# yeyupiaoling/VoiceprintRecognition-PaddlePaddle

Measured on NVIDIA H100. Metric: utterances/sec ECAPA-TDNN Fbank80 3s embed extract, higher is better.
Workload: dtype bf16x3 (split-bf16 operands, fp32 accumulate; fp32-grade)

## Files before the change

voiceprintrecognition-paddlepaddle_b200/csrc/asp_fused.cu:

```cuda
#include <stdio.h>
#include <string.h>

#include "common.h"
#include "ptx.cuh"

namespace ppv {

constexpr int AF_NT = 64;
constexpr int AF_A_TILE = 128 * 64 * 2;
constexpr int AF_B_TILE = AF_NT * 64 * 2;
constexpr int AF_X_TILE = AF_NT * 128 * 2;
constexpr int AF_STAGES = 2;
constexpr float LOG2E = 1.4426950408889634f;

template <int NSPLIT>
__global__ void __launch_bounds__(384, 1) asp_fused_kernel(const __grid_constant__ AspFusedParams p) {
    constexpr int NP = (NSPLIT == 3) ? 2 : 1;
    extern __shared__ uint8_t smem_raw[];
    const uint32_t smem_base = (smem_u32(smem_raw) + 1023u) & ~1023u;
    uint8_t* smem_gen = smem_raw + (smem_base - smem_u32(smem_raw));
    const int ksteps = p.K / 64;
    const int a_bytes = ksteps * NP * AF_A_TILE;
    const int b_bytes = ksteps * NP * AF_B_TILE;
    const int stage_bytes = b_bytes + 2 * AF_X_TILE;
    const uint32_t a_base = smem_base;
    const uint32_t s_base = smem_base + a_bytes;
    const uint32_t bar_base = s_base + AF_STAGES * stage_bytes;
    const uint32_t a_full = bar_base, a_empty = bar_base + 8;
    auto b_full = [&](int s) { return bar_base + 16u + 8u * s; };
    auto b_empty = [&](int s) { return bar_base + 32u + 8u * s; };

    const int warp = threadIdx.x >> 5, lane = threadIdx.x & 31;
    if (warp == 0 && lane == 0) {
        prefetch_tmap(&p.mapW);
        prefetch_tmap(&p.mapAtt);
        prefetch_tmap(&p.mapX);
    }
    if (warp == 1 && lane == 0) {
        mbar_init(a_full, 1);
        mbar_init(a_empty, 256);
        for (int s = 0; s < AF_STAGES; ++s) {
            mbar_init(b_full(s), 1);
            mbar_init(b_empty(s), 256);
        }
        fence_mbar_init();
    }
    __syncthreads();
    griddep_launch_dependents();
    griddep_wait();

    const int slabs = p.C / 128;
    const int items = slabs * p.B;
    const int ntiles = (p.T + AF_NT - 1) / AF_NT;

    if (warp == 0) {
        int stage = 0;
        uint32_t phase = 0, a_phase = 0;
        int cur_slab = -1;
        for (int item = blockIdx.x; item < items; item += gridDim.x) {
            const int b = item / slabs, slab = item - b * slabs;
            if (slab != cur_slab) {
                mbar_wait(a_empty, a_phase ^ 1u);
                if (lane == 0) {
                    mbar_arrive_expect_tx(a_full, a_bytes);
                    for (int ks = 0; ks < ksteps; ++ks)
                        for (int pl = 0; pl < NP; ++pl)
                            tma_load_3d(a_base + (ks * NP + pl) * AF_A_TILE, &p.mapW, a_full, ks * 64, slab * 128, pl);
                }
                __syncwarp();
                a_phase ^= 1u;
                cur_slab = slab;
            }
            {
                const int nitem = item + gridDim.x;
                if (nitem < items && lane < 2 * ntiles) {
                    const int nb = nitem / slabs, nslab = nitem - nb * slabs;
                    tma_prefetch_l2_3d(&p.mapX, nslab * 128, nb * p.Tp + p.P + (lane >> 1) * AF_NT, lane & 1);
                }
                __syncwarp();
            }
            const int row0 = b * p.Tp + p.P;
            for (int ft = 0; ft < ntiles; ++ft) {
                mbar_wait(b_empty(stage), phase ^ 1u);
                if (lane == 0) {
                    const uint32_t sb = s_base + stage * stage_bytes;
                    mbar_arrive_expect_tx(b_full(stage), stage_bytes);
                    for (int ks = 0; ks < ksteps; ++ks)
                        for (int pl = 0; pl < NP; ++pl)
                            tma_load_3d(sb + (ks * NP + pl) * AF_B_TILE, &p.mapAtt, b_full(stage), ks * 64, row0 + ft * AF_NT, pl);
                    for (int pl = 0; pl < 2; ++pl)
                        tma_load_3d(sb + b_bytes + pl * AF_X_TILE, &p.mapX, b_full(stage), slab * 128, row0 + ft * AF_NT, pl);
                }
                __syncwarp();
                if (++stage == AF_STAGES) {
                    stage = 0;
                    phase ^= 1u;
                }
            }
        }
    } else if (warp >= 4) {
        const int g = (warp - 4) >> 2, t = threadIdx.x & 127, w = t >> 5, l = t & 31;
        const int cl0 = 64 * g + 16 * w + (l >> 2);
        float acc[AF_NT / 2];
#pragma unroll
        for (int i = 0; i < AF_NT / 2; ++i) acc[i] = 0.f;
        int stage = 0;
        uint32_t phase = 0, a_phase = 0;
        int cur_slab = -1;
        for (int item = blockIdx.x; item < items; item += gridDim.x) {
            const int b = item / slabs, slab = item - b * slabs;
            if (slab != cur_slab) {
                mbar_wait(a_full, a_phase);
                a_phase ^= 1u;
                cur_slab = slab;
            }
            const int nitem = item + gridDim.x;
            const bool last_of_slab = (nitem >= items) || (nitem % slabs != slab);
            float m[2], S0[2], mu[2], M2[2];
#pragma unroll
            for (int rr = 0; rr < 2; ++rr) {
                m[rr] = -INFINITY;
                S0[rr] = mu[rr] = M2[rr] = 0.f;
            }
            const int Tb = p.nvalid ? max(1, min(p.T, p.nvalid[b])) : p.T;
            for (int ft = 0; ft < ntiles; ++ft) {
                mbar_wait(b_full(stage), phase);
                const uint32_t sb = s_base + stage * stage_bytes;
                wgmma_fence_acc(acc);
                wgmma_fence();
                for (int ks = 0; ks < ksteps; ++ks) {
                    const uint64_t a_hi = make_sw128_kmajor_desc(a_base + (ks * NP) * AF_A_TILE + g * 64 * 128);
                    const uint64_t b_hi = make_sw128_kmajor_desc(sb + (ks * NP) * AF_B_TILE);
#pragma unroll
                    for (int k = 0; k < 4; ++k) wgmma_bf16<AF_NT>(acc, a_hi + 2 * k, b_hi + 2 * k, (ks > 0 || k > 0) ? 1u : 0u);
                    if (NSPLIT == 3) {
                        const uint64_t a_lo = make_sw128_kmajor_desc(a_base + (ks * NP + 1) * AF_A_TILE + g * 64 * 128);
                        const uint64_t b_lo = make_sw128_kmajor_desc(sb + (ks * NP + 1) * AF_B_TILE);
#pragma unroll
                        for (int k = 0; k < 4; ++k) wgmma_bf16<AF_NT>(acc, a_lo + 2 * k, b_hi + 2 * k, 1u);
#pragma unroll
                        for (int k = 0; k < 4; ++k) wgmma_bf16<AF_NT>(acc, a_hi + 2 * k, b_lo + 2 * k, 1u);
                    }
                }
                wgmma_commit();
                wgmma_wait<0>();
                wgmma_fence_acc(acc);
                if (ft == ntiles - 1 && last_of_slab) mbar_arrive(a_empty);
                const __nv_bfloat16* xs_hi = reinterpret_cast<const __nv_bfloat16*>(smem_gen + (sb - smem_base) + b_bytes);
                const __nv_bfloat16* xs_lo = xs_hi + AF_X_TILE / 2;
                const int f0 = ft * AF_NT;
#pragma unroll
                for (int rr = 0; rr < 2; ++rr) {
                    float cm = -INFINITY;
#pragma unroll
                    for (int i = 0; i < AF_NT / 8; ++i)
#pragma unroll
                        for (int e = 0; e < 2; ++e)
                            if (f0 + 8 * i + 2 * (l & 3) + e < Tb) cm = fmaxf(cm, acc[4 * i + 2 * rr + e]);
                    if (cm > m[rr]) {
                        const float r = exp2f((m[rr] - cm) * LOG2E);
                        S0[rr] *= r;
                        M2[rr] *= r;
                        m[rr] = cm;
                    }
                    const float ms = m[rr] * LOG2E;
                    const int cl = cl0 + 8 * rr;
                    const float x0 = __bfloat162float(xs_hi[2 * (l & 3) * 128 + cl]) + __bfloat162float(xs_lo[2 * (l & 3) * 128 + cl]);
                    float xr[AF_NT / 8][2];
                    float wt = 0.f, sx = 0.f;
#pragma unroll
                    for (int i = 0; i < AF_NT / 8; ++i)
#pragma unroll
                        for (int e = 0; e < 2; ++e) {
                            const int fl = 8 * i + 2 * (l & 3) + e;
                            if (f0 + fl < Tb) {
                                const int o = fl * 128 + cl;
                                xr[i][e] = __bfloat162float(xs_hi[o]) + __bfloat162float(xs_lo[o]);
                                const float ev = exp2f(fmaf(acc[4 * i + 2 * rr + e], LOG2E, -ms));
                                acc[4 * i + 2 * rr + e] = ev;
                                wt += ev;
                                sx = fmaf(ev, xr[i][e] - x0, sx);
                            }
                        }
                    if (wt > 0.f) {
                        const float mt = x0 + sx / wt;
                        float m2 = 0.f;
#pragma unroll
                        for (int i = 0; i < AF_NT / 8; ++i)
#pragma unroll
                            for (int e = 0; e < 2; ++e)
                                if (f0 + 8 * i + 2 * (l & 3) + e < Tb) {
                                    const float d = xr[i][e] - mt;
                                    m2 = fmaf(acc[4 * i + 2 * rr + e] * d, d, m2);
                                }
                        const float n = S0[rr] + wt, f = wt / n, dl = mt - mu[rr];
                        mu[rr] = fmaf(dl, f, mu[rr]);
                        M2[rr] += m2 + dl * dl * (S0[rr] * f);
                        S0[rr] = n;
                    }
                }
                mbar_arrive(b_empty(stage));
                if (++stage == AF_STAGES) {
                    stage = 0;
                    phase ^= 1u;
                }
            }
#pragma unroll
            for (int rr = 0; rr < 2; ++rr) {
#pragma unroll
                for (int off = 1; off <= 2; off <<= 1) {
                    const float om = __shfl_xor_sync(0xffffffffu, m[rr], off), o0 = __shfl_xor_sync(0xffffffffu, S0[rr], off),
                                omu = __shfl_xor_sync(0xffffffffu, mu[rr], off), o2 = __shfl_xor_sync(0xffffffffu, M2[rr], off);
                    const float mm = fmaxf(m[rr], om);
                    const float ra = S0[rr] > 0.f ? exp2f((m[rr] - mm) * LOG2E) : 0.f, rb = o0 > 0.f ? exp2f((om - mm) * LOG2E) : 0.f;
                    const float wa = S0[rr] * ra, wb = o0 * rb, n = wa + wb;
                    const float f = n > 0.f ? wb / n : 0.f, dl = omu - mu[rr];
                    mu[rr] = fmaf(dl, f, mu[rr]);
                    M2[rr] = M2[rr] * ra + o2 * rb + dl * dl * (wa * f);
                    S0[rr] = n;
                    m[rr] = mm;
                }
            }
            if ((l & 3) != 0) continue;
            const int C = p.C;
#pragma unroll
            for (int rr = 0; rr < 2; ++rr) {
                const int c = slab * 128 + cl0 + 8 * rr;
                const float mean = mu[rr];
                const float sd = sqrtf(fmaxf(M2[rr] / S0[rr], p.eps));
                if (p.out_raw) {
                    p.out_raw[int64_t(b) * 2 * C + c] = mean;
                    p.out_raw[int64_t(b) * 2 * C + C + c] = sd;
                }
                __nv_bfloat16 h, lo;
                split_bf16(fmaf(mean, p.bn_scale[c], p.bn_shift[c]), h, lo);
                p.out.hi()[int64_t(b) * p.out.ld + c] = h;
                p.out.lo()[int64_t(b) * p.out.ld + c] = lo;
                split_bf16(fmaf(sd, p.bn_scale[C + c], p.bn_shift[C + c]), h, lo);
                p.out.hi()[int64_t(b) * p.out.ld + C + c] = h;
                p.out.lo()[int64_t(b) * p.out.ld + C + c] = lo;
            }
        }
    }
}

int asp_fused_build(AspFusedParams* p, const Planes& W, const Planes& att, const Planes& x, const float* bn_scale,
                    const float* bn_shift, const Planes& out, float* out_raw, int B, int T, int P, int Tp, int C, int K, float eps) {
    PPV_REQUIRE(C % 128 == 0 && K % 64 == 0 && K <= 128, "asp_fused: C % 128 == 0 and K in {64,128} required");
    memset(p, 0, sizeof(*p));
    PPV_REQUIRE(x.ld == C, "asp_fused: x row length must equal C");
    int rc = encode_planes_map(&p->mapW, W, 128);
    if (rc) return rc;
    rc = encode_planes_map(&p->mapAtt, att, AF_NT);
    if (rc) return rc;
    rc = encode_planes_map_ex(&p->mapX, x, 128, AF_NT, 0);
    if (rc) return rc;
    p->x = x;
    p->bn_scale = bn_scale;
    p->bn_shift = bn_shift;
    p->out = out;
    p->out_raw = out_raw;
    p->B = B;
    p->T = T;
    p->P = P;
    p->Tp = Tp;
    p->C = C;
    p->K = K;
    p->eps = eps;
    p->nvalid = nullptr;
    return PPV_OK;
}

int asp_fused_launch(const AspFusedParams& p, int precision, int num_sms, cudaStream_t st) {
    const bool x3 = precision == PPV_PREC_BF16X3;
    const int ksteps = p.K / 64, np = x3 ? 2 : 1;
    const int smem = 1024 + ksteps * np * AF_A_TILE + AF_STAGES * (ksteps * np * AF_B_TILE + 2 * AF_X_TILE) + 96 + 128 * 16 + 64;
    static bool attr3 = false, attr1 = false;
    bool& attr = x3 ? attr3 : attr1;
    if (!attr) {
        if (x3)
            PPV_CUDA_OK(cudaFuncSetAttribute(asp_fused_kernel<3>, cudaFuncAttributeMaxDynamicSharedMemorySize, 227 * 1024));
        else
            PPV_CUDA_OK(cudaFuncSetAttribute(asp_fused_kernel<1>, cudaFuncAttributeMaxDynamicSharedMemorySize, 227 * 1024));
        attr = true;
    }
    const int items = (p.C / 128) * p.B;
    const int grid = std::min(items, num_sms);
    if (x3)
        PPV_PDL_OK(launch_pdl(asp_fused_kernel<3>, dim3(grid), dim3(384), size_t(smem), st, p), "asp_fused_kernel");
    else
        PPV_PDL_OK(launch_pdl(asp_fused_kernel<1>, dim3(grid), dim3(384), size_t(smem), st, p), "asp_fused_kernel");
    return PPV_OK;
}

}
```

voiceprintrecognition-paddlepaddle_b200/csrc/capi.cu:

```cuda
#include <string.h>

#include <new>

#include "common.h"
#include "image_plan.h"
#include "model_common.h"

namespace ppv {

static thread_local std::string g_last_error;

void set_error(const std::string& msg) { g_last_error = msg; }
int fail(int code, const std::string& msg) {
    g_last_error = msg;
    return code;
}

int device_sm_count() {
    int dev = 0, n = 0;
    if (cudaGetDevice(&dev) != cudaSuccess || cudaDeviceGetAttribute(&n, cudaDevAttrMultiProcessorCount, dev) != cudaSuccess || n <= 0) {
        cudaGetLastError();
        return 132;
    }
    return n;
// ... 469 lines not shown
    rc = gemm_test_stage(A, W, M, N, K, ws, st, &pa, &pw);
    if (rc) return rc;
    GemmSource src{pa, 0, pa.ld, 0};
    const Planes po{static_cast<__nv_bfloat16*>(out), 0, N, int64_t(M) * N};
    Epilogue ep = Tp > 0 ? planes_epilogue(po, 0, Tp, P, Tp - 2 * P) : planes_epilogue(po);
    ep.bias = bias;
    ep.rowgrp_bias = rowgrp_bias;
    ep.relu = relu;
    ep.tanh_ = tanh_;
    ep.bn_scale = bn_scale;
    ep.bn_shift = bn_shift;
    GemmParams gp;
    rc = gemm_build(&gp, &src, 1, pw, M, N, ep, block_n, 64);
    if (rc) return rc;
    return gemm_launch(gp, precision, device_sm_count(), st);
    PPV_GUARD_END
}

static size_t conv2d_test_x_bytes(int B, int H, int W, int x_ld) {
    return au(au(size_t(B) * (H + 2) * (W + 2), 128) * size_t(x_ld) * 4, 256);
}
size_t ppv_conv2d_test_workspace_bytes(int B, int H, int W, int Cin, int Cout, int k, int x_ld) {
    if (x_ld <= 0) x_ld = Cin;
    return conv2d_test_x_bytes(B, H, W, x_ld) + au(au(size_t(Cout), 256) * k * k * Cin * 4, 256) + 256;
}
int ppv_conv2d_test(const float* x, const float* w, const float* bias, int relu, int B, int H, int W, int Cin, int Cout, int k,
                    int stride_h, int stride_w, int x_col0, int x_ld, int path, int precision, void* out, void* ws, size_t ws_bytes,
                    void* stream) {
    PPV_GUARD_BEGIN
    PPV_REQUIRE(x && w && out && ws, "ppv_conv2d_test: null argument");
    if (x_ld <= 0) x_ld = Cin;
    PPV_REQUIRE(B > 0 && H > 0 && W > 0 && Cin > 0 && Cout > 0 && (k == 1 || k == 3) && stride_h >= 1 && stride_w >= 1,
                "ppv_conv2d_test: bad shape");
    PPV_REQUIRE(x_col0 >= 0 && x_col0 + Cin <= x_ld, "ppv_conv2d_test: the input columns exceed x_ld");
    PPV_REQUIRE(path >= 0 && path <= 2, "ppv_conv2d_test: path must be 0 (3x3 patch kernel), 1 (pointwise kernel) or 2 (gather-GEMM)");
    PPV_REQUIRE(precision == PPV_PREC_BF16X3 || precision == PPV_PREC_BF16, "ppv_conv2d_test: bad precision");
    PPV_REQUIRE(ws_bytes >= ppv_conv2d_test_workspace_bytes(B, H, W, Cin, Cout, k, x_ld), "ppv_conv2d_test: workspace too small");
    const int Hp = H + 2, Wp = W + 2, Ho = (H - 1) / stride_h + 1, Wo = (W - 1) / stride_w + 1;
    const int64_t M = int64_t(B) * Hp * Wp;
    PPV_REQUIRE(M < (int64_t(1) << 31) && Wp + 1 < 32768, "ppv_conv2d_test: grid too large for 32-bit rows / 16-bit tap offsets");
    int rc = check_device();
    if (rc) return rc;
    cudaStream_t st = static_cast<cudaStream_t>(stream);
    Planes xp;
    xp.rows = int64_t(au(size_t(M), 128));
    xp.ld = x_ld;
    xp.plane_stride = xp.rows * x_ld;
    xp.base = static_cast<__nv_bfloat16*>(ws);
    const size_t x_bytes = conv2d_test_x_bytes(B, H, W, x_ld);
    PPV_CUDA_OK(cudaMemsetAsync(ws, 0, x_bytes, st));
    const size_t pitch = size_t(x_ld) * sizeof(__nv_bfloat16), rows2 = size_t(2 * xp.rows);
    if (x_col0 > 0) PPV_CUDA_OK(cudaMemset2DAsync(xp.base, pitch, 0x3f, size_t(x_col0) * sizeof(__nv_bfloat16), rows2, st));
    if (x_col0 + Cin < x_ld)
        PPV_CUDA_OK(cudaMemset2DAsync(xp.base + x_col0 + Cin, pitch, 0x3f, size_t(x_ld - x_col0 - Cin) * sizeof(__nv_bfloat16), rows2, st));
    for (int b = 0; b < B; ++b)
        for (int h = 0; h < H; ++h) {
            Planes row = xp;
            row.base = xp.base + ((int64_t(b) * Hp + h + 1) * Wp + 1) * x_ld + x_col0;
            rc = launch_f32_to_planes(x + (int64_t(b) * H + h) * W * Cin, W, Cin, row, st);
            if (rc) return rc;
        }
    const int K = k * k * Cin;
    std::vector<float> wh(size_t(Cout) * K);
    PPV_CUDA_OK(cudaMemcpyAsync(wh.data(), w, wh.size() * sizeof(float), cudaMemcpyDeviceToHost, st));
    PPV_CUDA_OK(cudaStreamSynchronize(st));
    ArenaBuilder ab;
    GemmWeights gw;
    ab.put_matrix(&gw, conv_weight_matrix(wh.data(), Cout, Cin, k * k, Cout, {{k * k, Cin, 0, Cin, 0}}), Cout, K);
    uint8_t* wdev = static_cast<uint8_t*>(ws) + x_bytes;
    PPV_CUDA_OK(cudaMemcpyAsync(wdev, ab.host.data(), ab.host.size(), cudaMemcpyHostToDevice, st));
    PPV_CUDA_OK(cudaStreamSynchronize(st));
    gw.W.base = reinterpret_cast<__nv_bfloat16*>(wdev + ab.patches[0].off);
    const int64_t out_plane = int64_t(B) * (Ho + 2) * (Wo + 2) * Cout;
    PPV_CUDA_OK(cudaMemsetAsync(out, 0, size_t(2 * out_plane) * sizeof(__nv_bfloat16), st));
    Planes outp;
    outp.base = static_cast<__nv_bfloat16*>(out);
    outp.ld = Cout;
    outp.plane_stride = out_plane;
    const ImageGeo gin{H, W, Hp, Wp}, gout{Ho, Wo, Ho + 2, Wo + 2};
    Epilogue ep = image_epilogue(outp, gin, gout, stride_h, stride_w);
    ep.bias = bias;
    ep.relu = relu ? 1 : 0;
    const int sms = device_sm_count();
    if (path == 0) {
        PPV_REQUIRE(k == 3 && conv3x3_c32_supported(Cin, Cout, H, W), "ppv_conv2d_test: the patch kernel takes 3x3 convs with 32 -> 32 channels only");
        Conv3x3Params cp;
        rc = conv3x3_build(&cp, xp, x_col0, gw.W, B, H, W, Hp, Wp, ep);
        if (rc) return rc;
        return conv3x3_launch(cp, precision, sms, st);
    }
    if (path == 1) {
        PPV_REQUIRE(k == 1, "ppv_conv2d_test: the pointwise kernel takes 1x1 convs only");
        const GemmSource src{xp, x_col0, Cin, 0};
        PwStep s;
        if (!pointwise_step_build(&s, &src, 1, gw.W, Cout, M, ep))
            return fail(PPV_EINVAL, "ppv_conv2d_test: the pointwise kernel does not take this conv (or PPV_POINTWISE=0)");
        return pointwise_launch(s, sms, st);
    }
    std::vector<GemmSource> srcs;
    if (k == 3)
        image_taps(&srcs, xp, x_col0, Cin, gin);
    else
        srcs.push_back(GemmSource{xp, x_col0, Cin, 0});
    GemmParams gp;
    rc = gemm_build(&gp, srcs.data(), int(srcs.size()), gw.W, int(M), Cout, ep, gemm_pick_bn(Cout));
    if (rc) return rc;
    return gemm_launch(gp, precision, sms, st);
    PPV_GUARD_END
}

static size_t asp_test_sizes(int B, int Tp, int C, int K, size_t* off) {
    const size_t rows = size_t(B) * Tp + 64;
    const size_t sz[4] = {size_t(C) * K, rows * K, rows * C, size_t(B) * 2 * C};
    size_t o = 0;
    for (int i = 0; i < 4; ++i) {
        off[i] = o;
        o += au(2 * sz[i] * sizeof(__nv_bfloat16), 256);
    }
    return o;
}
size_t ppv_asp_fused_test_workspace_bytes(int B, int Tp, int C, int K) {
    size_t off[4];
    return asp_test_sizes(B, Tp, C, K, off);
}
int ppv_asp_fused_test(const float* W, const float* att, const float* x, const float* bn_scale, const float* bn_shift,
                       const int* nvalid, int B, int T, int P, int Tp, int C, int K, int precision, int max_ctas, float* out_raw,
                       float* out, void* ws, size_t ws_bytes, void* stream) {
    PPV_GUARD_BEGIN
    PPV_REQUIRE(W && att && x && bn_scale && bn_shift && out_raw && out && ws, "ppv_asp_fused_test: null argument");
    PPV_REQUIRE(B > 0 && T > 0 && P >= 0 && Tp >= T + 2 * P && max_ctas >= 0, "ppv_asp_fused_test: bad shape");
    PPV_REQUIRE(precision == PPV_PREC_BF16X3 || precision == PPV_PREC_BF16, "ppv_asp_fused_test: bad precision");
    size_t off[4];
    PPV_REQUIRE(ws_bytes >= asp_test_sizes(B, Tp, C, K, off), "ppv_asp_fused_test: workspace too small");
    int rc = check_device();
    if (rc) return rc;
    cudaStream_t st = static_cast<cudaStream_t>(stream);
    uint8_t* w8 = static_cast<uint8_t*>(ws);
    const int64_t rows = int64_t(B) * Tp;
    auto planes = [&](int i, int64_t nrows, int ld, int64_t alloc_rows) {
        return Planes{reinterpret_cast<__nv_bfloat16*>(w8 + off[i]), nrows, ld, alloc_rows * ld};
    };
    const Planes pw = planes(0, C, K, C), pa = planes(1, rows, K, rows + 64), px = planes(2, rows, C, rows + 64),
                 po = planes(3, B, 2 * C, B);
    PPV_CUDA_OK(cudaMemsetAsync(w8 + off[1], 0x46, off[3] - off[1], st));
    if ((rc = launch_f32_to_planes(W, C, K, pw, st)) || (rc = launch_f32_to_planes(att, rows, K, pa, st)) ||
        (rc = launch_f32_to_planes(x, rows, C, px, st)))
        return rc;
    AspFusedParams ap;
    rc = asp_fused_build(&ap, pw, pa, px, bn_scale, bn_shift, po, out_raw, B, T, P, Tp, C, K, 1e-12f);
    if (rc) return rc;
    ap.nvalid = nvalid;
    rc = asp_fused_launch(ap, precision, max_ctas > 0 ? max_ctas : device_sm_count(), st);
    if (rc) return rc;
    return launch_planes_to_f32(po, 0, 2 * C, B, 1, 0, 1, out, st);
    PPV_GUARD_END
}

int ppv_gemm_bench(int M, int N, int K, int block_n, int block_k, int precision, int planes_out, int iters, void* ws, size_t ws_bytes,
                   float* ms_per_launch, void* stream) {
    PPV_GUARD_BEGIN
    PPV_REQUIRE(ws && ms_per_launch && iters > 0, "ppv_gemm_bench: bad argument");
    PPV_REQUIRE(planes_out >= 0 && planes_out <= 3, "ppv_gemm_bench: planes_out must be 0-3");
    constexpr int kTp = 306, kP = 4;
    PPV_REQUIRE(planes_out < 2 || M % kTp == 0, "ppv_gemm_bench: model epilogues need M % 306 == 0");
    cudaStream_t st = static_cast<cudaStream_t>(stream);
    const size_t Kp = au(size_t(K), 64);
    const size_t a_bytes = au(au(size_t(M), 128) * Kp * 4, 256), w_bytes = au(au(size_t(N), 256) * Kp * 4, 256);
    const size_t o_bytes = au(au(size_t(M), 128) * size_t(N) * 4, 256);
    const size_t v_bytes = au((3 + size_t(M / kTp)) * size_t(N) * 4, 256);
    PPV_REQUIRE(ws_bytes >= a_bytes + w_bytes + o_bytes + v_bytes, "ppv_gemm_bench: workspace too small");
    Planes pa, pw, po;
    pa.rows = int64_t(au(size_t(M), 128)); pa.ld = int(Kp); pa.plane_stride = pa.rows * pa.ld; pa.base = static_cast<__nv_bfloat16*>(ws);
    pw.rows = int64_t(au(size_t(N), 256)); pw.ld = int(Kp); pw.plane_stride = pw.rows * pw.ld;
    pw.base = reinterpret_cast<__nv_bfloat16*>(static_cast<uint8_t*>(ws) + a_bytes);
    po.rows = pa.rows; po.ld = N; po.plane_stride = po.rows * po.ld;
    po.base = reinterpret_cast<__nv_bfloat16*>(static_cast<uint8_t*>(ws) + a_bytes + w_bytes);
    PPV_CUDA_OK(cudaMemsetAsync(ws, 0x11, a_bytes + w_bytes, st));
    float* vec = reinterpret_cast<float*>(static_cast<uint8_t*>(ws) + a_bytes + w_bytes + o_bytes);
    PPV_CUDA_OK(cudaMemsetAsync(vec, 0x3c, v_bytes, st));
    GemmSource src{pa, 0, int(Kp), 0};
    Epilogue ep;
    if (planes_out >= 2) {
        ep = planes_epilogue(po, 0, kTp, kP, kTp - 2 * kP);
        ep.bias = vec; ep.bn_scale = vec + N; ep.bn_shift = vec + 2 * N;
        if (planes_out == 3) { ep.rowgrp_bias = vec + 3 * N; ep.tanh_ = 1; }
    } else if (planes_out) {
        ep = planes_epilogue(po);
    } else {
        ep.out_mode = OUT_F32; ep.out = po.base; ep.out_ld = N;
    }
    ep.relu = 1;
    GemmParams gp;
    int rc = gemm_build(&gp, &src, 1, pw, M, N, ep, block_n, block_k);
    if (rc) return rc;
    const int sms = device_sm_count();
    for (int i = 0; i < 3; ++i) { rc = gemm_launch(gp, precision, sms, st); if (rc) return rc; }
    cudaEvent_t e0, e1;
    PPV_CUDA_OK(cudaEventCreate(&e0));
    PPV_CUDA_OK(cudaEventCreate(&e1));
    PPV_CUDA_OK(cudaEventRecord(e0, st));
    for (int i = 0; i < iters; ++i) { rc = gemm_launch(gp, precision, sms, st); if (rc) return rc; }
    PPV_CUDA_OK(cudaEventRecord(e1, st));
    PPV_CUDA_OK(cudaEventSynchronize(e1));
    float ms = 0.f;
    PPV_CUDA_OK(cudaEventElapsedTime(&ms, e0, e1));
    cudaEventDestroy(e0);
    cudaEventDestroy(e1);
    gemm_trace_dump(gp);
    *ms_per_launch = ms / float(iters);
    return PPV_OK;
    PPV_GUARD_END
}

}
```

voiceprintrecognition-paddlepaddle_b200/csrc/common.h:

```cpp
#pragma once
#include <cuda.h>
#include <cuda_bf16.h>
#include <cuda_runtime.h>
#include <stdint.h>
#include <stdlib.h>

#include <algorithm>
#include <string>
#include <utility>

#include "../../include/ppv_b200.h"

namespace ppv {

void set_error(const std::string& msg);
int fail(int code, const std::string& msg);

#define PPV_CUDA_OK(expr)                                                                             \
    do {                                                                                              \
        cudaError_t _e = (expr);                                                                      \
        if (_e != cudaSuccess)                                                                        \
            return ::ppv::fail(PPV_ECUDA, std::string(#expr) + ": " + cudaGetErrorString(_e));        \
    } while (0)
#define PPV_LAUNCH_OK(what)                                                                           \
// ... 74 lines not shown
    const float* bias = nullptr;
    const float* rowgrp_bias = nullptr;
    const float* bn_scale = nullptr;
    const float* bn_shift = nullptr;
    int relu = 0;
    int tanh_ = 0;
    int sigmoid_ = 0;
    int silu_ = 0;
    float relu_max = 0.f;
    int out_mode = OUT_PLANES;
    void* out = nullptr;
    int64_t out_ld = 0;
    int64_t out_plane_stride = 0;
    int out_col0 = 0;
    int Tp = 0, P = 0, T = 0;
    int halo = 0;
    int img_Hp = 0, img_Wp = 0, img_H = 0, img_W = 0, img_stride = 1, out_Hp = 0, out_Wp = 0;
    int img_stride_w = 0;
    const float* seg_scale = nullptr;
    int seg_len = 0, nseg = 0;
    int zero_invalid = 0;
    int f32_vec_ok = 0;
    int debug_nostore = 0;
    int lean = 0;
};

inline Epilogue planes_epilogue(const Planes& out, int col0 = 0, int Tp = 0, int P = 0, int T = 0) {
    Epilogue ep;
    ep.out_mode = OUT_PLANES;
    ep.out = out.base;
    ep.out_ld = out.ld;
    ep.out_plane_stride = out.plane_stride;
    ep.out_col0 = col0;
    ep.Tp = Tp;
    ep.P = P;
    ep.T = T;
    return ep;
}

constexpr int GEMM_TRACE_TILES = 16;
constexpr int GEMM_TRACE_EVENTS = 16;

struct GemmParams {
    CUtensorMap mapA[GEMM_MAX_MAPS];
    CUtensorMap mapB;
    KStep ksteps[GEMM_MAX_KSTEPS];
    int num_ksteps;
    int bk;
    int ws;
    int lin_splits;
    int lin_b_row0, lin_b_col0;
    int64_t lin_split_rows;
    int M, N;
    int m_tiles, n_tiles;
    Epilogue epi;
    unsigned long long* trace;
    int trace_cta;
    int bn;
};
void gemm_trace_dump(const GemmParams& gp);

struct GemmSource {
    Planes t;
    int col0;
    int ncols;
    int row_off;
};

int gemm_build(GemmParams* gp, const GemmSource* srcs, int nsrc, const Planes& W, int M, int N, const Epilogue& epi,
               int BN, int BK = 0);
int gemm_build_wgrad(GemmParams* gp, const Planes& At, const Planes& Bt, int M, int N, int b_row0, int b_col0, int splits, float* out,
                     int64_t out_ld, int out_col0, int64_t split_rows, int BN);
int gemm_launch(const GemmParams& gp, int precision, int num_sms, cudaStream_t stream);
inline int gemm_pick_bn(int N, int max_bn = 256) {
    for (int bn = max_bn; bn > 64; bn /= 2)
        if (N % bn == 0) return bn;
    return 64;
}

int encode_planes_map(CUtensorMap* m, const Planes& t, int box_rows);
int encode_planes_map_ex(CUtensorMap* m, const Planes& t, int box_cols, int box_rows, int swizzle_bytes);

struct Res2Params {
    CUtensorMap mapA[2];
    CUtensorMap mapW;
    int a_col[2];
    int nsrc, dil;
    int l2_prefetch;
    int M, m_tiles;
    Epilogue epi;
};
int res2conv_build(Res2Params* rp, const GemmSource* srcs, int nsrc, const Planes& W, int M, int dil, const Epilogue& epi);
int res2conv_launch(const Res2Params& rp, int precision, int num_sms, cudaStream_t st);

struct Conv3x3Params {
    CUtensorMap mapX;
    CUtensorMap mapW;
    int x_col0;
    int B, H, W, Hp, Wp;
    int nph, npw, patches;
    Epilogue epi;
};
bool conv3x3_c32_supported(int Cin, int Cout, int H, int W);
int conv3x3_build(Conv3x3Params* cp, const Planes& x, int x_col0, const Planes& Wt, int B, int H, int W, int Hp, int Wp, const Epilogue& epi);
int conv3x3_launch(const Conv3x3Params& cp, int precision, int num_sms, cudaStream_t st);

constexpr int RES2CHAIN_MAX = 7;
struct Res2ChainParams {
    CUtensorMap mapX;
    CUtensorMap mapXt, mapY, mapYtail;
    CUtensorMap mapW[RES2CHAIN_MAX];
    const float* bias[RES2CHAIN_MAX];
    const float* bn_scale[RES2CHAIN_MAX];
    const float* bn_shift[RES2CHAIN_MAX];
    Planes x;
    Planes y;
    int nconv, width, B, T, P, Tp, dil, ntiles;
    int paired;
    unsigned long long* trace;
};
int res2chain_build(Res2ChainParams* cp, const Planes& x, const Planes& y, const Planes* W, const float* const* bias, const float* const* bn_scale,
                    const float* const* bn_shift, int nconv, int B, int T, int P, int Tp, int dil, bool paired);
int res2chain_launch(const Res2ChainParams& cp, int precision, int num_sms, cudaStream_t st);
bool res2chain_fits(int T, int P);
bool res2chain_pair_fits(int T, int P);
void res2chain_trace_dump(const Res2ChainParams& cp);

int pointwise_launch(const GemmSource* srcs, int nsrc, const Planes& W, int64_t M, int N, const Epilogue& ep, int num_sms, cudaStream_t st);
struct PwStep {
    GemmSource srcs[2];
    int nsrc = 0, N = 0;
    int64_t M = 0;
    Planes W;
    Epilogue ep;
};
inline int pointwise_launch(const PwStep& s, int num_sms, cudaStream_t st) { return pointwise_launch(s.srcs, s.nsrc, s.W, s.M, s.N, s.ep, num_sms, st); }
bool pointwise_step_build(PwStep* s, const GemmSource* srcs, int nsrc, const Planes& W, int N, int64_t M, const Epilogue& ep);

bool skinny_linear_supported(int M, int N, int K, const Epilogue& ep);
int skinny_linear_launch(const Planes& x, int x_col0, const Planes& W, int M, int N, int K, const Epilogue& ep, cudaStream_t st);

struct AspFusedParams {
    CUtensorMap mapW;
    CUtensorMap mapAtt;
    CUtensorMap mapX;
    Planes x;
    const float* bn_scale;
    const float* bn_shift;
    Planes out;
    float* out_raw;
    int B, T, P, Tp, C, K;
    float eps;
    const int* nvalid;
};

int asp_fused_build(AspFusedParams* p, const Planes& W, const Planes& att, const Planes& x, const float* bn_scale,
                    const float* bn_shift, const Planes& out, float* out_raw, int B, int T, int P, int Tp, int C, int K, float eps);
int asp_fused_launch(const AspFusedParams& p, int precision, int num_sms, cudaStream_t st);

int launch_pack_features(const float* feat, int B, int T, int F, const Planes& out, int P, int Tp, cudaStream_t st);
int launch_colstats(const Planes& x, int col0, int C, int B, int T, int P, int Tp, int mode, float eps, float* out_f32,
                    const Planes& out_pl, cudaStream_t st, float inv_count = 0.f, const int* nvalid = nullptr);
int launch_lengths_to_counts(const float* lengths, int B, int T, int* nvalid, cudaStream_t st);
int launch_se_scale_res(const Planes& z, const float* scale, const Planes& res, int rc0, const Planes& out, int oc0, int C,
                        int Tp, int64_t rows, int num_sms, cudaStream_t st, int relu = 0, float relu_max = 0.f);
int launch_asp_pool(const float* logits, int64_t lg_ld, const Planes& x, int C, int B, int T, int P, int Tp, float eps,
                    const float* bn_scale, const float* bn_shift, const Planes& out_pl, float* out_raw, cudaStream_t st);
int launch_planes_to_f32(const Planes& x, int col0, int C, int B, int T, int P, int Tp, float* out, cudaStream_t st);
int launch_f32_to_planes(const float* src, int64_t rows, int cols, const Planes& out, cudaStream_t st);

struct Fbank;
int fbank_create(const ppv_fbank_cfg* cfg, Fbank** out);
void fbank_destroy(Fbank* h);
int fbank_num_frames(const Fbank* h, int L);
int fbank_n_mels(const Fbank* h);
int fbank_run(Fbank* h, const float* wav, const float* lens_ratio, int B, int L, float* raw, float* out_f32,
              const Planes& out_pl, int P, int Tp, cudaStream_t st, const int* valid_frames = nullptr);

size_t audio_prep_workspace_bytes(int B, int max_new_len);
int audio_prep(const float* wav, int64_t wav_ld, const int32_t* iparams, const float* fparams, const float* noise, int B, int max_new_len,
               float target_db, int normalize, int Lout, float* out, void* ws, size_t ws_bytes, cudaStream_t st);
size_t audio_prep_reverb_workspace_bytes(int B, int max_new_len, int max_rir_len);
int audio_prep_reverb(const float* wav, int64_t wav_ld, const int32_t* iparams, const float* fparams, const float* noise, const float* rir_bank,
                      int64_t rir_bank_len, const int32_t* rparams, int B, int max_new_len, int max_rir_len, float target_db, int normalize,
                      int Lout, float* out, void* ws, size_t ws_bytes, cudaStream_t st);

size_t reverb_workspace_bytes(int B, int max_new_len, int max_rir_len);
int reverb_run(const float* wav, int64_t wav_ld, const int32_t* iparams, const float* fparams, const float* noise, const float* rir_bank,
               int64_t rir_bank_len, const int32_t* rparams, int B, int max_new_len, int max_rir_len, float target_db, int normalize,
               int Lout, float* out, float* gains, void* ws, cudaStream_t st);

struct Spectral;
void spectral_default_cfg(ppv_spectral_cfg* c, int method);
int spectral_create(const ppv_spectral_cfg* cfg, Spectral** out);
void spectral_destroy(Spectral* h);
int spectral_num_frames(const Spectral* h, int L);
int spectral_feature_dim(const Spectral* h);
int spectral_run(Spectral* h, const float* wav, const float* lens_ratio, int B, int L, float* out, cudaStream_t st);
int spec_augment_run(float* feat, const int32_t* params, int B, int T, int F, int n_freq_masks, int n_time_masks, int fill_mode, cudaStream_t st);

struct Model;
void ppv_ecapa_default_cfg_impl(ppv_ecapa_cfg* c);
int ecapa_create(const ppv_ecapa_cfg* cfg, Model** out);
int ecapa_forward(Model* m, const float* feat, Fbank* fb, const float* wav, const float* lens_ratio, int B, int T, int L, float* emb,
                  void* ws, size_t ws_bytes, cudaStream_t st, const float* lengths = nullptr);
int ecapa_profile(Model* m, int enable);
int ecapa_profile_read(Model* m, double* gemm_ms, double* other_ms, int64_t* gemm_launches, int64_t* other_launches);
void ppv_resnetse_default_cfg_impl(ppv_resnetse_cfg* c);
int resnetse_create(const ppv_resnetse_cfg* cfg, Model** out);
void ppv_eres2net_default_cfg_impl(ppv_eres2net_cfg* c);
int eres2net_create(const ppv_eres2net_cfg* cfg, Model** out);
void ppv_campplus_default_cfg_impl(ppv_campplus_cfg* c);
int campplus_create(const ppv_campplus_cfg* cfg, Model** out);

struct ImageGeo {
    int H = 0, W = 0, Hp = 0, Wp = 0;
    int64_t rows(int B) const { return int64_t(B) * Hp * Wp; }
};
int launch_stem_conv(const float* feat, int B, int T, int F, const float* w9, const float* bias, int C0, const Planes& out, int Hp, int Wp,
                     cudaStream_t st);
int launch_flatten_image(const Planes& in, int B, int H, int W, int Hp, int Wp, int C, const Planes& out, int num_sms, cudaStream_t st);
int launch_image_to_f32(const Planes& in, int B, int H, int W, int Hp, int Wp, int C, float* out, cudaStream_t st);
int launch_aff_combine(const Planes& x, int xc0, const Planes& y, int yc0, const Planes& t, const Planes& out, int C, int64_t rows, int num_sms,
                       cudaStream_t st);

struct Trainer;
int trainer_create(const ppv_ecapa_cfg* cfg, int num_classes, Trainer** out);
void trainer_destroy(Trainer* t);
int64_t trainer_param_count(const Trainer* t);
int64_t trainer_stat_count(const Trainer* t);
int trainer_lookup(const Trainer* t, const char* name, int64_t* off, int64_t* numel, int* is_stat);
int trainer_bind(Trainer* t, float* params, float* grads, float* stats);
int trainer_set_precision(Trainer* t, int precision);
size_t trainer_workspace_bytes(const Trainer* t, int B, int T);
int trainer_forward_backward(Trainer* t, const float* feat, const int64_t* labels, int B, int T, float margin, float scale, int easy_margin,
                             float label_smoothing, float* loss_out, float* logits_out, void* ws, size_t ws_bytes, cudaStream_t st);
int trainer_read_tap(Trainer* t, const char* name, float* out, size_t out_elems, cudaStream_t st);
int adam_step(float* params, const float* grads, float* m, float* v, int64_t n, float lr, float beta1, float beta2, float eps, float weight_decay,
              int64_t step, float grad_scale, cudaStream_t st);

size_t cosine_workspace_bytes(int M, int N, int D);
int cosine_matrix(const float* A, const float* Bm, int M, int N, int D, float* out, void* ws, size_t ws_bytes, int precision,
                  cudaStream_t st);
int cosine_pairlist(const float* E, const int32_t* idx, int64_t P, int n, int D, float* out, cudaStream_t st);
size_t aam_workspace_bytes(int B, int D, int S);
int aam_forward(const float* emb, const float* W, const int64_t* labels, int B, int D, int S, float margin, float scale,
                int easy_margin, float label_smoothing, float* logits, float* loss, void* ws, size_t ws_bytes, cudaStream_t st);
int aam_backward(const float* emb, const float* W, const int64_t* labels, const float* logits, int B, int D, int S, float margin,
                 float scale, int easy_margin, float label_smoothing, float* d_emb, float* d_W, void* ws, size_t ws_bytes,
                 cudaStream_t st);

size_t eer_workspace_bytes(int64_t n);
int eer_mindcf(const float* scores, const int32_t* labels, const int32_t* row_labels, const int32_t* col_labels, int ncols, int64_t n,
               double p_target, double c_miss, double c_fa, double* out, void* ws, size_t ws_bytes, cudaStream_t st);
int row_argmax(const float* sim, int rows, int cols, int32_t* idx, float* best, cudaStream_t st);

int cluster_prune(float* A, int N, double pval, cudaStream_t st);
int cluster_laplacian(const float* P, int N, double* L, cudaStream_t st);
size_t sym_eig_workspace_bytes(int N, int m);
int sym_eig_smallest(double* L, int N, int m, double* evals, double* evecs, void* ws, size_t ws_bytes, cudaStream_t st);
size_t kmeans_workspace_bytes(int N, int k);
int kmeans(const double* X, int ld, int N, int k, const double* uniforms, int n_uniforms, int max_iter, int32_t* labels, double* inertia, void* ws,
           size_t ws_bytes, cudaStream_t st);

int device_sm_count();

}
```

Baseline: 47240.

## Swizzle ASP x tile loads, add full-tile fast path, hoist BN params, add tracing

Splits each x-tile TMA load into two 64-column boxes using a 128-byte swizzle and computes matching XOR-swizzled shared-memory offsets. The goal is to avoid bank conflicts when the epilogue reads x by channel. The per-tile softmax-moment epilogue becomes a templated helper with a branch-free path for tiles that are fully valid. BN scale and shift values are loaded once per item, and the L2 prefetch is adjusted to the new box shape. An env-gated clock64 tracing facility is also added; it costs only a branch and predicated stores when disabled.

```diff
diff --git a/voiceprintrecognition-paddlepaddle_b200/csrc/asp_fused.cu b/voiceprintrecognition-paddlepaddle_b200/csrc/asp_fused.cu
--- a/voiceprintrecognition-paddlepaddle_b200/csrc/asp_fused.cu
+++ b/voiceprintrecognition-paddlepaddle_b200/csrc/asp_fused.cu
@@ -1,4 +1,5 @@
 #include <stdio.h>
+#include <stdlib.h>
 #include <string.h>
 
 #include "common.h"
@@ -10,8 +11,57 @@
 constexpr int AF_A_TILE = 128 * 64 * 2;
 constexpr int AF_B_TILE = AF_NT * 64 * 2;
 constexpr int AF_X_TILE = AF_NT * 128 * 2;
+constexpr int AF_X_BOX = AF_X_TILE / 2;
 constexpr int AF_STAGES = 2;
 constexpr float LOG2E = 1.4426950408889634f;
+
+template <bool FULL>
+__device__ __forceinline__ void asp_tile_moments(float (&acc)[AF_NT / 2], int rr, const __nv_bfloat16* xs_hi, const __nv_bfloat16* xs_lo,
+                                                 const int (&xo)[2], int f0, int q, int Tb, float& m, float& S0, float& mu, float& M2) {
+    float cm = -INFINITY;
+#pragma unroll
+    for (int i = 0; i < AF_NT / 8; ++i)
+#pragma unroll
+        for (int e = 0; e < 2; ++e)
+            cm = fmaxf(cm, (FULL || f0 + 8 * i + 2 * q + e < Tb) ? acc[4 * i + 2 * rr + e] : -INFINITY);
+    if (cm > m) {
+        const float r = exp2f((m - cm) * LOG2E);
+        S0 *= r;
+        M2 *= r;
+        m = cm;
+    }
+    const float ms = m * LOG2E;
+    const float x0 = __bfloat162float(xs_hi[xo[0]]) + __bfloat162float(xs_lo[xo[0]]);
+    float xr[AF_NT / 8][2];
+    float wt = 0.f, sx = 0.f;
+#pragma unroll
+    for (int i = 0; i < AF_NT / 8; ++i)
+#pragma unroll
+        for (int e = 0; e < 2; ++e) {
+            const bool v = FULL || f0 + 8 * i + 2 * q + e < Tb;
+            const int o = xo[e] + 512 * i;
+            xr[i][e] = v ? __bfloat162float(xs_hi[o]) + __bfloat162float(xs_lo[o]) : x0;
+            const float ev = v ? exp2f(fmaf(acc[4 * i + 2 * rr + e], LOG2E, -ms)) : 0.f;
+            acc[4 * i + 2 * rr + e] = ev;
+            wt += ev;
+            sx = fmaf(ev, xr[i][e] - x0, sx);
+        }
+    if (wt > 0.f) {
+        const float mt = x0 + sx / wt;
+        float m2 = 0.f;
+#pragma unroll
+        for (int i = 0; i < AF_NT / 8; ++i)
+#pragma unroll
+            for (int e = 0; e < 2; ++e) {
+                const float d = xr[i][e] - mt;
+                m2 = fmaf(acc[4 * i + 2 * rr + e] * d, d, m2);
+            }
+        const float n = S0 + wt, f = wt / n, dl = mt - mu;
+        mu = fmaf(dl, f, mu);
+        M2 += m2 + dl * dl * (S0 * f);
+        S0 = n;
+    }
+}
 
 template <int NSPLIT>
 __global__ void __launch_bounds__(384, 1) asp_fused_kernel(const __grid_constant__ AspFusedParams p) {
@@ -31,6 +81,11 @@
     auto b_empty = [&](int s) { return bar_base + 32u + 8u * s; };
 
     const int warp = threadIdx.x >> 5, lane = threadIdx.x & 31;
+    const bool trace_cta = p.trace != nullptr && int(blockIdx.x) == p.trace_cta;
+    auto stamp = [&](bool on, int role, int tile, int ev) {
+        if (on && tile < ASP_TRACE_TILES) p.trace[(role * ASP_TRACE_TILES + tile) * ASP_TRACE_EVENTS + ev] = clock64();
+    };
+    stamp(trace_cta && threadIdx.x == 0, 0, 0, 7);
     if (warp == 0 && lane == 0) {
         prefetch_tmap(&p.mapW);
         prefetch_tmap(&p.mapAtt);
@@ -56,7 +111,7 @@
     if (warp == 0) {
         int stage = 0;
         uint32_t phase = 0, a_phase = 0;
-        int cur_slab = -1;
+        int cur_slab = -1, lt = 0;
         for (int item = blockIdx.x; item < items; item += gridDim.x) {
             const int b = item / slabs, slab = item - b * slabs;
             if (slab != cur_slab) {
@@ -73,23 +128,27 @@
             }
             {
                 const int nitem = item + gridDim.x;
-                if (nitem < items && lane < 2 * ntiles) {
+                if (nitem < items && lane < 4 * ntiles) {
                     const int nb = nitem / slabs, nslab = nitem - nb * slabs;
-                    tma_prefetch_l2_3d(&p.mapX, nslab * 128, nb * p.Tp + p.P + (lane >> 1) * AF_NT, lane & 1);
+                    tma_prefetch_l2_3d(&p.mapX, nslab * 128 + (lane & 2) * 32, nb * p.Tp + p.P + (lane >> 2) * AF_NT, lane & 1);
                 }
                 __syncwarp();
             }
             const int row0 = b * p.Tp + p.P;
-            for (int ft = 0; ft < ntiles; ++ft) {
+            for (int ft = 0; ft < ntiles; ++ft, ++lt) {
                 mbar_wait(b_empty(stage), phase ^ 1u);
                 if (lane == 0) {
+                    stamp(trace_cta, 0, lt, 0);
                     const uint32_t sb = s_base + stage * stage_bytes;
                     mbar_arrive_expect_tx(b_full(stage), stage_bytes);
                     for (int ks = 0; ks < ksteps; ++ks)
                         for (int pl = 0; pl < NP; ++pl)
                             tma_load_3d(sb + (ks * NP + pl) * AF_B_TILE, &p.mapAtt, b_full(stage), ks * 64, row0 + ft * AF_NT, pl);
                     for (int pl = 0; pl < 2; ++pl)
-                        tma_load_3d(sb + b_bytes + pl * AF_X_TILE, &p.mapX, b_full(stage), slab * 128, row0 + ft * AF_NT, pl);
+                        for (int h = 0; h < 2; ++h)
+                            tma_load_3d(sb + b_bytes + pl * AF_X_TILE + h * AF_X_BOX, &p.mapX, b_full(stage), slab * 128 + h * 64,
+                                        row0 + ft * AF_NT, pl);
+                    stamp(trace_cta, 0, lt, 1);
                 }
                 __syncwarp();
                 if (++stage == AF_STAGES) {
@@ -99,8 +158,15 @@
             }
         }
     } else if (warp >= 4) {
-        const int g = (warp - 4) >> 2, t = threadIdx.x & 127, w = t >> 5, l = t & 31;
+        const int g = (warp - 4) >> 2, t = threadIdx.x & 127, w = t >> 5, l = t & 31, q = l & 3;
         const int cl0 = 64 * g + 16 * w + (l >> 2);
+        int xo[2][2];
+#pragma unroll
+        for (int rr = 0; rr < 2; ++rr)
+#pragma unroll
+            for (int e = 0; e < 2; ++e) xo[rr][e] = g * (AF_X_BOX / 2) + (2 * q + e) * 64 + (((2 * w + rr) ^ (2 * q + e)) << 3) + (l >> 2);
+        const bool tr = trace_cta && t == 0;
+        int lt = 0;
         float acc[AF_NT / 2];
 #pragma unroll
         for (int i = 0; i < AF_NT / 2; ++i) acc[i] = 0.f;
@@ -123,8 +189,19 @@
                 S0[rr] = mu[rr] = M2[rr] = 0.f;
             }
             const int Tb = p.nvalid ? max(1, min(p.T, p.nvalid[b])) : p.T;
-            for (int ft = 0; ft < ntiles; ++ft) {
+            float bn[2][4];
+#pragma unroll
+            for (int rr = 0; rr < 2; ++rr) {
+                const int c = slab * 128 + cl0 + 8 * rr;
+                bn[rr][0] = p.bn_scale[c];
+                bn[rr][1] = p.bn_shift[c];
+                bn[rr][2] = p.bn_scale[p.C + c];
+                bn[rr][3] = p.bn_shift[p.C + c];
+            }
+            for (int ft = 0; ft < ntiles; ++ft, ++lt) {
+                stamp(tr, 1 + g, lt, 0);
                 mbar_wait(b_full(stage), phase);
+                stamp(tr, 1 + g, lt, 1);
                 const uint32_t sb = s_base + stage * stage_bytes;
                 wgmma_fence_acc(acc);
                 wgmma_fence();
@@ -143,63 +220,23 @@
                     }
                 }
                 wgmma_commit();
+                stamp(tr, 1 + g, lt, 2);
                 wgmma_wait<0>();
                 wgmma_fence_acc(acc);
+                stamp(tr, 1 + g, lt, 3);
                 if (ft == ntiles - 1 && last_of_slab) mbar_arrive(a_empty);
                 const __nv_bfloat16* xs_hi = reinterpret_cast<const __nv_bfloat16*>(smem_gen + (sb - smem_base) + b_bytes);
                 const __nv_bfloat16* xs_lo = xs_hi + AF_X_TILE / 2;
                 const int f0 = ft * AF_NT;
 #pragma unroll
                 for (int rr = 0; rr < 2; ++rr) {
-                    float cm = -INFINITY;
-#pragma unroll
-                    for (int i = 0; i < AF_NT / 8; ++i)
-#pragma unroll
-                        for (int e = 0; e < 2; ++e)
-                            if (f0 + 8 * i + 2 * (l & 3) + e < Tb) cm = fmaxf(cm, acc[4 * i + 2 * rr + e]);
-                    if (cm > m[rr]) {
-                        const float r = exp2f((m[rr] - cm) * LOG2E);
-                        S0[rr] *= r;
-                        M2[rr] *= r;
-                        m[rr] = cm;
-                    }
-                    const float ms = m[rr] * LOG2E;
-                    const int cl = cl0 + 8 * rr;
-                    const float x0 = __bfloat162float(xs_hi[2 * (l & 3) * 128 + cl]) + __bfloat162float(xs_lo[2 * (l & 3) * 128 + cl]);
-                    float xr[AF_NT / 8][2];
-                    float wt = 0.f, sx = 0.f;
-#pragma unroll
-                    for (int i = 0; i < AF_NT / 8; ++i)
-#pragma unroll
-                        for (int e = 0; e < 2; ++e) {
-                            const int fl = 8 * i + 2 * (l & 3) + e;
-                            if (f0 + fl < Tb) {
-                                const int o = fl * 128 + cl;
-                                xr[i][e] = __bfloat162float(xs_hi[o]) + __bfloat162float(xs_lo[o]);
-                                const float ev = exp2f(fmaf(acc[4 * i + 2 * rr + e], LOG2E, -ms));
-                                acc[4 * i + 2 * rr + e] = ev;
-                                wt += ev;
-                                sx = fmaf(ev, xr[i][e] - x0, sx);
-                            }
-                        }
-                    if (wt > 0.f) {
-                        const float mt = x0 + sx / wt;
-                        float m2 = 0.f;
-#pragma unroll
-                        for (int i = 0; i < AF_NT / 8; ++i)
-#pragma unroll
-                            for (int e = 0; e < 2; ++e)
-                                if (f0 + 8 * i + 2 * (l & 3) + e < Tb) {
-                                    const float d = xr[i][e] - mt;
-                                    m2 = fmaf(acc[4 * i + 2 * rr + e] * d, d, m2);
-                                }
-                        const float n = S0[rr] + wt, f = wt / n, dl = mt - mu[rr];
-                        mu[rr] = fmaf(dl, f, mu[rr]);
-                        M2[rr] += m2 + dl * dl * (S0[rr] * f);
-                        S0[rr] = n;
-                    }
+                    if (f0 + AF_NT <= Tb)
+                        asp_tile_moments<true>(acc, rr, xs_hi, xs_lo, xo[rr], f0, q, Tb, m[rr], S0[rr], mu[rr], M2[rr]);
+                    else
+                        asp_tile_moments<false>(acc, rr, xs_hi, xs_lo, xo[rr], f0, q, Tb, m[rr], S0[rr], mu[rr], M2[rr]);
                 }
                 mbar_arrive(b_empty(stage));
+                stamp(tr, 1 + g, lt, 4);
                 if (++stage == AF_STAGES) {
                     stage = 0;
                     phase ^= 1u;
@@ -233,10 +270,10 @@
                     p.out_raw[int64_t(b) * 2 * C + C + c] = sd;
                 }
                 __nv_bfloat16 h, lo;
-                split_bf16(fmaf(mean, p.bn_scale[c], p.bn_shift[c]), h, lo);
+                split_bf16(fmaf(mean, bn[rr][0], bn[rr][1]), h, lo);
                 p.out.hi()[int64_t(b) * p.out.ld + c] = h;
                 p.out.lo()[int64_t(b) * p.out.ld + c] = lo;
-                split_bf16(fmaf(sd, p.bn_scale[C + c], p.bn_shift[C + c]), h, lo);
+                split_bf16(fmaf(sd, bn[rr][2], bn[rr][3]), h, lo);
                 p.out.hi()[int64_t(b) * p.out.ld + C + c] = h;
                 p.out.lo()[int64_t(b) * p.out.ld + C + c] = lo;
             }
@@ -253,7 +290,7 @@
     if (rc) return rc;
     rc = encode_planes_map(&p->mapAtt, att, AF_NT);
     if (rc) return rc;
-    rc = encode_planes_map_ex(&p->mapX, x, 128, AF_NT, 0);
+    rc = encode_planes_map_ex(&p->mapX, x, 64, AF_NT, 128);
     if (rc) return rc;
     p->x = x;
     p->bn_scale = bn_scale;
@@ -268,7 +305,39 @@
     p->K = K;
     p->eps = eps;
     p->nvalid = nullptr;
+    if (const char* tr = getenv("PPV_ASP_TRACE")) {
+        constexpr size_t n = 3 * ASP_TRACE_TILES * ASP_TRACE_EVENTS;
+        static unsigned long long* buf = nullptr;
+        if (!buf) PPV_CUDA_OK(cudaMalloc(reinterpret_cast<void**>(&buf), n * sizeof(unsigned long long)));
+        PPV_CUDA_OK(cudaMemset(buf, 0, n * sizeof(unsigned long long)));
+        p->trace = buf;
+        p->trace_cta = atoi(tr);
+    }
     return PPV_OK;
+}
+
+void asp_trace_dump(const AspFusedParams& p) {
+    if (!p.trace) return;
+    constexpr int E = ASP_TRACE_EVENTS;
+    unsigned long long h[3 * ASP_TRACE_TILES * E];
+    cudaDeviceSynchronize();
+    cudaMemcpy(h, p.trace, sizeof(h), cudaMemcpyDeviceToHost);
+    const unsigned long long t0 = h[7];
+    auto at = [&](int r, int i, int e) -> long long { const unsigned long long v = h[(r * ASP_TRACE_TILES + i) * E + e]; return v ? (long long)(v - t0) : -1ll; };
+    printf("asp trace B=%d T=%d C=%d K=%d CTA %d (cycles from kernel start)\n", p.B, p.T, p.C, p.K, p.trace_cta);
+    long long prev[2] = {-1, -1};
+    for (int i = 0; i < ASP_TRACE_TILES; ++i) {
+        printf("asp trace tile %2d  tma slot %7lld issued %7lld", i, at(0, i, 0), at(0, i, 1));
+        for (int g = 0; g < 2; ++g) {
+            const int r = 1 + g;
+            if (at(r, i, 4) < 0) continue;
+            printf("  | wg%d full %7lld wait %5lld mma %5lld epi %5lld period %5lld", g, at(r, i, 1), at(r, i, 1) - at(r, i, 0),
+                   at(r, i, 3) - at(r, i, 1), at(r, i, 4) - at(r, i, 3), prev[g] >= 0 ? at(r, i, 4) - prev[g] : -1ll);
+            prev[g] = at(r, i, 4);
+        }
+        printf("\n");
+    }
+    fflush(stdout);
 }
 
 int asp_fused_launch(const AspFusedParams& p, int precision, int num_sms, cudaStream_t st) {
diff --git a/voiceprintrecognition-paddlepaddle_b200/csrc/capi.cu b/voiceprintrecognition-paddlepaddle_b200/csrc/capi.cu
--- a/voiceprintrecognition-paddlepaddle_b200/csrc/capi.cu
+++ b/voiceprintrecognition-paddlepaddle_b200/csrc/capi.cu
@@ -645,6 +645,7 @@
     ap.nvalid = nvalid;
     rc = asp_fused_launch(ap, precision, max_ctas > 0 ? max_ctas : device_sm_count(), st);
     if (rc) return rc;
+    asp_trace_dump(ap);
     return launch_planes_to_f32(po, 0, 2 * C, B, 1, 0, 1, out, st);
     PPV_GUARD_END
 }
diff --git a/voiceprintrecognition-paddlepaddle_b200/csrc/common.h b/voiceprintrecognition-paddlepaddle_b200/csrc/common.h
--- a/voiceprintrecognition-paddlepaddle_b200/csrc/common.h
+++ b/voiceprintrecognition-paddlepaddle_b200/csrc/common.h
@@ -250,7 +250,12 @@
     int B, T, P, Tp, C, K;
     float eps;
     const int* nvalid;
-};
+    unsigned long long* trace;
+    int trace_cta;
+};
+constexpr int ASP_TRACE_TILES = 16;
+constexpr int ASP_TRACE_EVENTS = 8;
+void asp_trace_dump(const AspFusedParams& p);
 
 int asp_fused_build(AspFusedParams* p, const Planes& W, const Planes& att, const Planes& x, const float* bn_scale,
                     const float* bn_shift, const Planes& out, float* out_raw, int B, int T, int P, int Tp, int C, int K, float eps);
```

Result: no change. 48040 (median of 6 runs) (+1.7%).
